# yangdongchao/RSTnet

Measured on NVIDIA H100. Metric: codec_frames_per_s, higher is better.
Workload: dtype f32

## Files before the change

### include/rstnet_b200.h

```cpp
#ifndef RSTNET_B200_H
#define RSTNET_B200_H

#include <stdint.h>

#ifdef __cplusplus
extern "C" {
#endif

typedef void* rstnet_stream_t;

enum { RSTNET_ACT_NONE = 0, RSTNET_ACT_ELU = 1, RSTNET_ACT_GELU = 2 };

int rstnet_version(void);
const char* rstnet_last_error(void);
int64_t rstnet_launch_count(void);
uint32_t rstnet_device_error_flags(int clear);

typedef struct {
  const float* A;
  int64_t a_batch_stride, a_row_stride;
  const float* Wt;
  const float* bias;
  const float* scale;
  const float* R;
// ... 7 lines not shown
} rstnet_gemm_rows_args;
int rstnet_gemm_rows_f32(const rstnet_gemm_rows_args* args, rstnet_stream_t stream);

typedef struct rstnet_tc_plan rstnet_tc_plan;
typedef struct {
  const float* A;
  int64_t a_i_stride, a_o_stride;
  int32_t a_c_extent, a_i_extent, a_o_extent;
  int32_t taps, tap_di, tap_do, o_mul;
  const float* W;
  const float* W_lo;
  int32_t N, Kc;
  int32_t I_out, O_out;
  float* C;
  int64_t c_i_stride, c_o_stride, c_split_stride;
  const float* R;
  int64_t r_i_stride, r_o_stride, r_split_stride;
  const float* bias;
  const float* scale;
  int32_t n_split;
  int32_t pre_act, post_act, precision;
  float* C2;
  int32_t act2;
} rstnet_tc_gemm_desc;
int rstnet_tc_gemm_create(const rstnet_tc_gemm_desc* desc, rstnet_tc_plan** out);
int rstnet_tc_gemm_run(const rstnet_tc_plan* plan, rstnet_stream_t stream);
void rstnet_tc_gemm_destroy(rstnet_tc_plan* plan);
int rstnet_tc_gemm_grid(const rstnet_tc_plan* plan, int32_t* grid_x, int32_t* grid_y, int32_t* tile_n);
typedef struct rstnet_tc_resblock_plan rstnet_tc_resblock_plan;
typedef struct {
  const float* Y;
  int64_t y_i_stride, y_o_stride;
  int32_t channels;
  int32_t I_out, O_out, y_rows;
  const float* W1;
  const float* W1_lo;
  const float* b1;
  const float* W2;
  const float* W2_lo;
  const float* b2;
  float* out;
  int64_t out_i_stride, out_o_stride;
} rstnet_tc_resblock_desc;
int rstnet_tc_resblock_create(const rstnet_tc_resblock_desc* desc, rstnet_tc_resblock_plan** out);
int rstnet_tc_resblock_run(const rstnet_tc_resblock_plan* plan, rstnet_stream_t stream);
void rstnet_tc_resblock_destroy(rstnet_tc_resblock_plan* plan);

int rstnet_tf32_split_f32(const float* x, float* hi, float* lo, int64_t n, rstnet_stream_t stream);

int rstnet_conv1d_cin1_f32(const float* x, int64_t x_batch_stride, int64_t x_time_stride, const float* w, const float* bias,
                           float* out, float* out2 , int64_t out_batch_stride,
// ... 131 lines not shown
```

### rstnet_b200/_lib.py

```python
from __future__ import annotations

import ctypes as C
import os

_HERE = os.path.dirname(os.path.abspath(__file__))
LIB_PATH = os.path.join(_HERE, "lib", "librstnet_b200.so")

ACT_NONE, ACT_ELU, ACT_GELU = 0, 1, 2

SYMBOLS = [
    "rstnet_version", "rstnet_last_error", "rstnet_launch_count", "rstnet_device_error_flags",
    "rstnet_gemm_rows_f32", "rstnet_tc_gemm_create", "rstnet_tc_gemm_run", "rstnet_tc_gemm_destroy", "rstnet_tc_gemm_grid",
    "rstnet_tc_resblock_create", "rstnet_tc_resblock_run", "rstnet_tc_resblock_destroy", "rstnet_tf32_split_f32", "rstnet_conv1d_cin1_f32", "rstnet_conv1d_cout1_f32",
    "rstnet_convtr1d_depthwise_f32", "rstnet_rows_fill_f32", "rstnet_rows_copy_table_f32",
    "rstnet_counter_add", "rstnet_layer_norm_f32", "rstnet_rope_kv_append_f32",
    "rstnet_ring_attention_f32", "rstnet_rope_ring_attention_f32", "rstnet_rvq_encode_workspace", "rstnet_rvq_encode_f32",
    "rstnet_rvq_decode_gather_f32",
    "rstnet_skinny_gemm_workspace", "rstnet_skinny_gemm_create", "rstnet_skinny_gemm_create_fused", "rstnet_skinny_gemm_run", "rstnet_skinny_gemm_destroy",
    "rstnet_lm_embed_sum_bf16", "rstnet_lm_embed_rows_bf16", "rstnet_lm_rms_norm_bf16", "rstnet_lm_rope_kv_append_bf16",
    "rstnet_lm_rope_pair_kv_append_bf16",
    "rstnet_lm_ring_decode_attention_bf16", "rstnet_lm_silu_mul_bf16", "rstnet_lm_depth_attention_bf16",
    "rstnet_resample_f32", "rstnet_lm_delay_cache_in", "rstnet_lm_delay_cache_out", "rstnet_counter_add_rows",
    "rstnet_lm_cross_entropy_bf16", "rstnet_rows_fill_tail_f32", "rstnet_lm_sample_params_bf16",
    "rstnet_lm_rope_kv_append_paged_bf16", "rstnet_lm_paged_decode_attention_bf16",
]

KV_LOG2_PAGE_MIN, KV_LOG2_PAGE_MAX = 4, 12

RESAMPLE_MAX_TABLE_BYTES = 48 * 1024


class GemmRowsArgs(C.Structure):
    _fields_ = [
        ("A", C.c_void_p), ("a_batch_stride", C.c_int64), ("a_row_stride", C.c_int64),
        ("Wt", C.c_void_p), ("bias", C.c_void_p), ("scale", C.c_void_p),
        ("R", C.c_void_p), ("r_batch_stride", C.c_int64), ("r_row_stride", C.c_int64),
        ("C", C.c_void_p), ("c_batch_stride", C.c_int64), ("c_row_stride", C.c_int64),
        ("batch", C.c_int32), ("rows", C.c_int32), ("N", C.c_int32), ("K", C.c_int32),
        ("pre_act", C.c_int32), ("post_act", C.c_int32), ("taps", C.c_int32), ("tap_stride", C.c_int64),
    ]


class TcGemmDesc(C.Structure):
    _fields_ = [
        ("A", C.c_void_p), ("a_i_stride", C.c_int64), ("a_o_stride", C.c_int64),
        ("a_c_extent", C.c_int32), ("a_i_extent", C.c_int32), ("a_o_extent", C.c_int32),
        ("taps", C.c_int32), ("tap_di", C.c_int32), ("tap_do", C.c_int32), ("o_mul", C.c_int32),
        ("W", C.c_void_p), ("W_lo", C.c_void_p), ("N", C.c_int32), ("Kc", C.c_int32), ("I_out", C.c_int32), ("O_out", C.c_int32),
        ("C", C.c_void_p), ("c_i_stride", C.c_int64), ("c_o_stride", C.c_int64), ("c_split_stride", C.c_int64),
        ("R", C.c_void_p), ("r_i_stride", C.c_int64), ("r_o_stride", C.c_int64), ("r_split_stride", C.c_int64),
        ("bias", C.c_void_p), ("scale", C.c_void_p),
        ("n_split", C.c_int32), ("pre_act", C.c_int32), ("post_act", C.c_int32), ("precision", C.c_int32),
        ("C2", C.c_void_p), ("act2", C.c_int32),
    ]


class TcResblockDesc(C.Structure):
    _fields_ = [
        ("Y", C.c_void_p), ("y_i_stride", C.c_int64), ("y_o_stride", C.c_int64),
        ("channels", C.c_int32), ("I_out", C.c_int32), ("O_out", C.c_int32), ("y_rows", C.c_int32),
        ("W1", C.c_void_p), ("W1_lo", C.c_void_p), ("b1", C.c_void_p),
        ("W2", C.c_void_p), ("W2_lo", C.c_void_p), ("b2", C.c_void_p),
        ("out", C.c_void_p), ("out_i_stride", C.c_int64), ("out_o_stride", C.c_int64),
    ]


class RowCopy(C.Structure):
    _fields_ = [("buf", C.c_void_p), ("batch_stride", C.c_int64), ("C", C.c_int32), ("src_row", C.c_int32),
                ("dst_row", C.c_int32), ("nrows", C.c_int32), ("cps", C.c_int32), ("reserved", C.c_int32)]


class RstnetError(RuntimeError):
    pass


_lib = None
# ... 4 lines not shown
    if _lib is not None:
        return _lib
    if not os.path.exists(LIB_PATH):
        raise RstnetError(
            f"{LIB_PATH} not found: the CUDA extension is not built. Run `python -m rstnet_b200.build` "
            "(there is no CPU fallback).")
    from . import build as _build
    stamp = os.path.join(os.path.dirname(LIB_PATH), "build.sha256")
    if os.path.isdir(_build.CSRC) and (not os.path.exists(stamp) or open(stamp).read().strip() != _build._digest()):
        raise RstnetError(
            f"{LIB_PATH} is stale (built from different sources than rstnet_b200/csrc + include/). "
            "Run `python -m rstnet_b200.build`.")
    L = C.CDLL(LIB_PATH)
    vp, i32, i64, f32 = C.c_void_p, C.c_int32, C.c_int64, C.c_float
    L.rstnet_version.restype = C.c_int
    L.rstnet_last_error.restype = C.c_char_p
    L.rstnet_launch_count.restype = i64
    L.rstnet_gemm_rows_f32.argtypes = [C.POINTER(GemmRowsArgs), vp]
    L.rstnet_tc_gemm_create.argtypes = [C.POINTER(TcGemmDesc), C.POINTER(C.c_void_p)]
    L.rstnet_tc_gemm_run.argtypes = [vp, vp]
    L.rstnet_tc_gemm_destroy.argtypes = [vp]
    L.rstnet_tc_gemm_destroy.restype = None
    L.rstnet_tc_gemm_grid.argtypes = [vp, C.POINTER(i32), C.POINTER(i32), C.POINTER(i32)]
    L.rstnet_tc_resblock_create.argtypes = [C.POINTER(TcResblockDesc), C.POINTER(C.c_void_p)]
    L.rstnet_tc_resblock_run.argtypes = [vp, vp]
    L.rstnet_tc_resblock_destroy.argtypes = [vp]
    L.rstnet_tc_resblock_destroy.restype = None
    L.rstnet_tf32_split_f32.argtypes = [vp, vp, vp, i64, vp]
    L.rstnet_conv1d_cin1_f32.argtypes = [vp, i64, i64, vp, vp, vp, vp, i64, i64, i32, i32, i32, i32, i32, i32, vp]
    L.rstnet_conv1d_cout1_f32.argtypes = [vp, i64, i64, vp, vp, vp, i64, i32, i32, i32, i32, vp]
    L.rstnet_convtr1d_depthwise_f32.argtypes = [vp, i64, i64, vp, vp, i64, i64, i32, i32, i32, i32, vp]
    L.rstnet_rows_fill_f32.argtypes = [vp, i64, i32, i32, i32, i32, i32, i32, vp, i32, i32, vp]
    L.rstnet_rows_fill_tail_f32.argtypes = [vp, i64, i32, i32, i32, i32, i32, vp, i64, i32, vp]
    L.rstnet_rows_copy_table_f32.argtypes = [vp, i32, i32, vp, vp]
    L.rstnet_counter_add.argtypes = [vp, i64, i32, vp, vp]
    L.rstnet_layer_norm_f32.argtypes = [vp, i64, vp, vp, vp, i32, i32, i32, f32, vp]
    L.rstnet_rope_kv_append_f32.argtypes = [vp, i64, i64, vp, vp, i32, vp, i32, i32, i32, i32, i32, vp]
    L.rstnet_ring_attention_f32.argtypes = [vp, i64, i64, vp, vp, i32, vp, i64, i64, i32, i32, i32, i32, i32, i32, i32, vp]
    L.rstnet_rope_ring_attention_f32.argtypes = [vp, i64, i64, vp, vp, i32, vp, vp, i64, i64, i32, i32, i32, i32, i32, i32, vp]
    L.rstnet_rvq_encode_workspace.argtypes = [i64, i32, i32, i32]
    L.rstnet_rvq_encode_workspace.restype = i64
    L.rstnet_rvq_encode_f32.argtypes = [vp, i64, vp, vp, vp, vp, vp, i64, i32, i32, i32, i32, i32, i32, vp]
    L.rstnet_rvq_decode_gather_f32.argtypes = [vp, vp, vp, i64, i32, i32, i32, i32, i32, i32, vp]
    L.rstnet_skinny_gemm_workspace.argtypes = [i32, i32, i32]
    L.rstnet_skinny_gemm_workspace.restype = i64
    L.rstnet_skinny_gemm_create.argtypes = [vp, vp, vp, vp, vp, i32, i32, i32, i32, C.POINTER(C.c_void_p)]
# ... 42 lines not shown
```

### rstnet_b200/csrc/gemm_tc.cu

```cuda
#include <cstdlib>

#include "common.cuh"
#include "tc_common.cuh"
#include "../../include/rstnet_b200.h"

namespace rstnet {
extern void count_launch();
using namespace tc;

constexpr int TC_BM = 128;
constexpr int TC_BKE = 32;
constexpr int TC_A_BYTES = TC_BM * 128;
constexpr int TC_CONSUMER_WARPS = 8;
constexpr int TC_THREADS = 32 * TC_CONSUMER_WARPS + 32;
constexpr int TC_CHUNK_STAGES = 4;

struct TcParams {
  float* C;
  float* C2;
  int act2;
  long long c_i_stride, c_o_stride, c_split_stride;
  const float* R;
  long long r_i_stride, r_o_stride, r_split_stride;
  const float* bias;
  const float* scale;
  int n_split;
  int I_out, O_out, N, Kc;
  int taps, tap_di, tap_do, o_mul, kchunks;
  int pre_act, post_act, i_tiles;
  int m_tiles, n_tiles;
};

template <int BN, int PREC>
struct TcCfg {
  static constexpr bool SPLIT = PREC == 0;
  static constexpr int B_BYTES = BN * 128;
  static constexpr int STAGE_BYTES = TC_A_BYTES + B_BYTES * (SPLIT ? 2 : 1);
  static constexpr int STAGES = (200 * 1024 / STAGE_BYTES) > 8 ? 8 : (200 * 1024 / STAGE_BYTES);
  static constexpr int SMEM_BYTES = STAGES * STAGE_BYTES + 1024  + 256 ;
};

__device__ __forceinline__ float tf32_rna(float x) {
  const uint32_t u = __float_as_uint(x);
  return __uint_as_float((x != x ? u | 0x00400000u : u + 0x1000u) & 0xFFFFE000u);
}
__device__ __forceinline__ float tf32_rna_lo(float x, float hi) {
  const float d = x - hi;
  return d != d ? 0.f : __uint_as_float((__float_as_uint(d) + 0x1000u) & 0xFFFFE000u);
}

__device__ __forceinline__ float act_tc(float x, int act) {
  if (act == ACT_ELU) return elu_fast(x);
  if (act == ACT_GELU) return gelu_f(x);
  return x;
}

template <bool SPLIT, bool PRE_ELU>
__device__ __forceinline__ void tc_build_a(uint32_t st, uint32_t a_row, uint32_t a_sw, uint32_t (&ah)[4][4], uint32_t (&al)[4][4]) {
#pragma unroll
  for (int k = 0; k < 4; ++k) {
#pragma unroll
    for (int e = 0; e < 4; ++e) {
// ... 134 lines not shown
          if (p.scale) {
            const float2 ss = *reinterpret_cast<const float2*>(p.scale + n);
            v.x *= ss.x; v.y *= ss.y;
          }
          long long coff = n, roff = n;
          if (p.n_split > 0) {
            const int j = n / p.n_split, co = n % p.n_split;
            coff = (long long)j * p.c_split_stride + co;
            roff = (long long)j * p.r_split_stride + co;
          }
          if (rrow) {
            const float2 rr = *reinterpret_cast<const float2*>(rrow + roff);
            v.x += rr.x; v.y += rr.y;
          }
          if (crow2)
            *reinterpret_cast<float2*>(crow2 + coff) = make_float2(act_tc(v.x, p.act2), act_tc(v.y, p.act2));
          *reinterpret_cast<float2*>(crow + coff) = make_float2(act_tc(v.x, p.post_act), act_tc(v.y, p.post_act));
        }
      }
    }
  }
}

constexpr int RB_B_BYTES = 64 * 128;
constexpr int RB_STAGE_BYTES = TC_A_BYTES + 2 * RB_B_BYTES;
constexpr int RB_STAGES = 6;

struct RbParams {
  float* out;
  long long o_i_stride, o_o_stride;
  const float* b1;
  const float* b2;
  int I_out, i_tiles, m_tiles;
};

template <int C>
struct RbCfg {
  static constexpr int N1 = C / 2;
  static constexpr int KCH = C / 32;
  static constexpr int P1 = 3 * KCH;
  static constexpr int NS = C / 64;
  static constexpr int K2 = N1 / 32;
  static constexpr int H_BYTES = K2 * TC_A_BYTES;
  static constexpr int SMEM_BYTES = RB_STAGES * RB_STAGE_BYTES + H_BYTES + 1024  + 256 ;
  static constexpr bool ring_ok() {
    for (int j = 0; j < NS; ++j)
// ... 178 lines not shown
                                  CUtensorMapL2promotion, CUtensorMapFloatOOBfill);

static EncodeTiledFn get_encode_fn() {
  static EncodeTiledFn fn = nullptr;
  if (!fn) {
    void* p = nullptr;
    cudaDriverEntryPointQueryResult q;
    if (cudaGetDriverEntryPoint("cuTensorMapEncodeTiled", &p, cudaEnableDefault, &q) == cudaSuccess && p) fn = (EncodeTiledFn)p;
  }
  return fn;
}

}
using namespace rstnet;

struct rstnet_tc_plan {
  CUtensorMap tmA, tmW, tmWlo;
  TcParams p;
  dim3 grid;
  int bn, prec;
};

template <int BN, int PREC, bool PRE_ELU>
static int tc_launch(const rstnet_tc_plan* pl, cudaStream_t st) {
  using Cfg = TcCfg<BN, PREC>;
  static unsigned long long attr = 0;
  smem_optin(gemm_tc_kernel<BN, PREC, PRE_ELU>, Cfg::SMEM_BYTES, attr);
  gemm_tc_kernel<BN, PREC, PRE_ELU><<<pl->grid, TC_THREADS, Cfg::SMEM_BYTES, st>>>(pl->tmA, pl->tmW, pl->tmWlo, pl->p);
  count_launch();
  return check_launch("gemm_tc");
}

extern "C" int rstnet_tc_gemm_create(const rstnet_tc_gemm_desc* d, rstnet_tc_plan** out) {
  RSTNET_REQUIRE(d && out, "tc_gemm_create: null argument");
  RSTNET_REQUIRE(d->A && d->W && d->C, "tc_gemm_create: null tensor pointer");
  RSTNET_REQUIRE(d->precision != 0 || d->W_lo, "tc_gemm_create: precision 0 (3xTF32) needs W_lo");
  RSTNET_REQUIRE(d->Kc > 0 && d->Kc % TC_BKE == 0, "tc_gemm_create: Kc (%d) must be a multiple of %d", d->Kc, TC_BKE);
  RSTNET_REQUIRE(d->N > 0 && d->N % 4 == 0, "tc_gemm_create: N (%d) must be a multiple of 4", d->N);
  RSTNET_REQUIRE(d->taps >= 1 && d->I_out > 0 && d->O_out > 0, "tc_gemm_create: bad shape");
  RSTNET_REQUIRE(d->precision == 0 || d->precision == 1, "tc_gemm_create: precision must be 0 (3xTF32) or 1 (TF32)");
  RSTNET_REQUIRE(d->pre_act == ACT_NONE || d->pre_act == ACT_ELU, "tc_gemm_create: pre_act must be NONE or ELU (got %d)", d->pre_act);
  RSTNET_REQUIRE((uintptr_t)d->A % 16 == 0 && (uintptr_t)d->W % 16 == 0 && (uintptr_t)d->C % 16 == 0 &&
                     d->a_i_stride % 4 == 0 && d->a_o_stride % 4 == 0 && d->c_i_stride % 4 == 0 && d->c_o_stride % 4 == 0 &&
                     d->c_split_stride % 4 == 0 && d->n_split % 4 == 0,
                 "tc_gemm_create: 16-byte alignment required");
  EncodeTiledFn enc = get_encode_fn();
  RSTNET_REQUIRE(enc != nullptr, "tc_gemm_create: cuTensorMapEncodeTiled unavailable (no CUDA driver?)");
  rstnet_tc_plan* pl = new rstnet_tc_plan();
  const int N = d->N;
  const int sms = sm_count();
  pl->bn = N >= 64 ? 64 : 32;
  const int i_tiles = ceil_div(d->I_out, TC_BM);
  {
    const long long mt = (long long)i_tiles * d->O_out;
    const long long t64 = mt * ceil_div(N, 64), t32 = mt * ceil_div(N, 32);
    if (pl->bn == 64 && ((t32 + sms - 1) / sms) * 2 <= ((t64 + sms - 1) / sms) * 3) pl->bn = 32;
  }
  pl->prec = d->precision;
  {
    cuuint64_t gdim[3] = {(cuuint64_t)d->a_c_extent, (cuuint64_t)d->a_i_extent, (cuuint64_t)d->a_o_extent};
    cuuint64_t gstr[2] = {(cuuint64_t)d->a_i_stride * 4, (cuuint64_t)d->a_o_stride * 4};
    cuuint32_t box[3] = {TC_BKE, TC_BM, 1};
    cuuint32_t estr[3] = {1, 1, 1};
    CUresult r = enc(&pl->tmA, CU_TENSOR_MAP_DATA_TYPE_FLOAT32, 3, (void*)d->A, gdim, gstr, box, estr, CU_TENSOR_MAP_INTERLEAVE_NONE,
                     CU_TENSOR_MAP_SWIZZLE_128B, CU_TENSOR_MAP_L2_PROMOTION_L2_128B, CU_TENSOR_MAP_FLOAT_OOB_FILL_NONE);
    if (r != CUDA_SUCCESS) {
      delete pl;
      set_error("tc_gemm_create: cuTensorMapEncodeTiled(A) failed with %d", (int)r);
      return 3;
    }
  }
  {
    cuuint64_t gdim[2] = {(cuuint64_t)d->taps * d->Kc, (cuuint64_t)N};
    cuuint64_t gstr[1] = {(cuuint64_t)d->taps * d->Kc * 4};
    cuuint32_t box[2] = {TC_BKE, (cuuint32_t)pl->bn};
    cuuint32_t estr[2] = {1, 1};
    CUresult r = enc(&pl->tmW, CU_TENSOR_MAP_DATA_TYPE_FLOAT32, 2, (void*)d->W, gdim, gstr, box, estr, CU_TENSOR_MAP_INTERLEAVE_NONE,
                     CU_TENSOR_MAP_SWIZZLE_128B, CU_TENSOR_MAP_L2_PROMOTION_L2_256B, CU_TENSOR_MAP_FLOAT_OOB_FILL_NONE);
    if (r == CUDA_SUCCESS && d->W_lo)
      r = enc(&pl->tmWlo, CU_TENSOR_MAP_DATA_TYPE_FLOAT32, 2, (void*)d->W_lo, gdim, gstr, box, estr, CU_TENSOR_MAP_INTERLEAVE_NONE,
              CU_TENSOR_MAP_SWIZZLE_128B, CU_TENSOR_MAP_L2_PROMOTION_L2_256B, CU_TENSOR_MAP_FLOAT_OOB_FILL_NONE);
    else
      pl->tmWlo = pl->tmW;
    if (r != CUDA_SUCCESS) {
      delete pl;
      set_error("tc_gemm_create: cuTensorMapEncodeTiled(W) failed with %d", (int)r);
      return 3;
    }
  }
  TcParams& p = pl->p;
  p.C2 = d->C2; p.act2 = d->act2;
  p.C = d->C; p.c_i_stride = d->c_i_stride; p.c_o_stride = d->c_o_stride; p.c_split_stride = d->c_split_stride;
  p.R = d->R; p.r_i_stride = d->r_i_stride; p.r_o_stride = d->r_o_stride; p.r_split_stride = d->r_split_stride;
  p.bias = d->bias; p.scale = d->scale; p.n_split = d->n_split;
  p.I_out = d->I_out; p.O_out = d->O_out; p.N = N; p.Kc = d->Kc;
  p.taps = d->taps; p.tap_di = d->tap_di; p.tap_do = d->tap_do; p.o_mul = d->o_mul; p.kchunks = d->Kc / TC_BKE;
  p.pre_act = d->pre_act; p.post_act = d->post_act; p.i_tiles = i_tiles;
  p.m_tiles = i_tiles * d->O_out;
  p.n_tiles = ceil_div(N, pl->bn);
  const long long tiles = (long long)p.m_tiles * p.n_tiles;
  pl->grid = dim3((unsigned)(tiles < sms ? tiles : sms));
  *out = pl;
  return 0;
}

extern "C" int rstnet_tc_gemm_run(const rstnet_tc_plan* pl, rstnet_stream_t stream) {
  RSTNET_REQUIRE(pl != nullptr, "tc_gemm_run: null plan");
  cudaStream_t st = (cudaStream_t)stream;
  const bool elu = pl->p.pre_act == ACT_ELU;
  if (pl->prec == 0) {
    if (pl->bn == 64) return elu ? tc_launch<64, 0, true>(pl, st) : tc_launch<64, 0, false>(pl, st);
    return elu ? tc_launch<32, 0, true>(pl, st) : tc_launch<32, 0, false>(pl, st);
  }
  if (pl->bn == 64) return elu ? tc_launch<64, 1, true>(pl, st) : tc_launch<64, 1, false>(pl, st);
  return elu ? tc_launch<32, 1, true>(pl, st) : tc_launch<32, 1, false>(pl, st);
}

extern "C" void rstnet_tc_gemm_destroy(rstnet_tc_plan* pl) { delete pl; }

struct rstnet_tc_resblock_plan {
  CUtensorMap tmY, tmW1, tmW1lo, tmW2, tmW2lo;
  RbParams p;
  dim3 grid;
  int channels;
// ... 54 lines not shown

template <int Cc>
static int rb_launch(const rstnet_tc_resblock_plan* pl, cudaStream_t st) {
  constexpr int smem = RbCfg<Cc>::SMEM_BYTES;
  static unsigned long long attr = 0;
  smem_optin(resblock_tc_kernel<Cc>, smem, attr);
  resblock_tc_kernel<Cc><<<pl->grid, TC_THREADS, smem, st>>>(pl->tmY, pl->tmW1, pl->tmW1lo, pl->tmW2, pl->tmW2lo, pl->p);
  count_launch();
  return check_launch("tc_resblock");
}

extern "C" int rstnet_tc_resblock_run(const rstnet_tc_resblock_plan* pl, rstnet_stream_t stream) {
  RSTNET_REQUIRE(pl != nullptr, "tc_resblock_run: null plan");
  cudaStream_t st = (cudaStream_t)stream;
  return pl->channels == 64 ? rb_launch<64>(pl, st) : rb_launch<128>(pl, st);
}

extern "C" void rstnet_tc_resblock_destroy(rstnet_tc_resblock_plan* pl) { delete pl; }
extern "C" int rstnet_tc_gemm_grid(const rstnet_tc_plan* pl, int32_t* gx, int32_t* gy, int32_t* bn) {
  if (!pl) return 1;
  *gx = pl->p.m_tiles; *gy = pl->p.n_tiles; *bn = pl->bn;
  return 0;
}

namespace rstnet {
__global__ void tf32_split_kernel(const float* __restrict__ x, float* __restrict__ hi, float* __restrict__ lo, long long n) {
  for (long long i = (long long)blockIdx.x * blockDim.x + threadIdx.x; i < n; i += (long long)gridDim.x * blockDim.x) {
    const float v = x[i], h = tf32_rna(v);
    hi[i] = h;
    lo[i] = tf32_rna_lo(v, h);
  }
}
}

extern "C" int rstnet_tf32_split_f32(const float* x, float* hi, float* lo, int64_t n, rstnet_stream_t stream) {
  RSTNET_REQUIRE(x && hi && lo, "tf32_split: null pointer");
  if (n <= 0) return 0;
  int g = ceil_div(n, 256);
  if (g > sm_count() * 8) g = sm_count() * 8;
  rstnet::tf32_split_kernel<<<g, 256, 0, (cudaStream_t)stream>>>(x, hi, lo, n);
  count_launch();
  return check_launch("tf32_split");
}
```

### rstnet_b200/csrc/tc_common.cuh

```cuda
#pragma once
#include <cuda.h>
#include <cuda_runtime.h>
#include <cstdint>

namespace rstnet {
namespace tc {

__device__ __forceinline__ uint32_t smem_u32(const void* p) { return static_cast<uint32_t>(__cvta_generic_to_shared(p)); }

__device__ __forceinline__ bool elect_one() {
  uint32_t pred = 0;
  asm volatile(
      "{\n\t.reg .b32 rx;\n\t.reg .pred px;\n\t"
      "elect.sync rx|px, 0xFFFFFFFF;\n\t"
      "selp.u32 %0, 1, 0, px;\n\t}"
      : "=r"(pred));
  return pred != 0;
}

__device__ __forceinline__ void mbar_init(uint64_t* bar, uint32_t count) {
  asm volatile("mbarrier.init.shared::cta.b64 [%0], %1;" ::"r"(smem_u32(bar)), "r"(count));
}
__device__ __forceinline__ void fence_barrier_init() { asm volatile("fence.mbarrier_init.release.cluster;" ::: "memory"); }
__device__ __forceinline__ void mbar_arrive(uint64_t* bar) {
  asm volatile("{\n\t.reg .b64 st;\n\tmbarrier.arrive.shared::cta.b64 st, [%0];\n\t}" ::"r"(smem_u32(bar)) : "memory");
}
__device__ __forceinline__ void mbar_arrive_expect_tx(uint64_t* bar, uint32_t bytes) {
  asm volatile("{\n\t.reg .b64 st;\n\tmbarrier.arrive.expect_tx.shared::cta.b64 st, [%0], %1;\n\t}" ::"r"(smem_u32(bar)), "r"(bytes)
               : "memory");
}
__device__ __forceinline__ bool mbar_try_wait(uint64_t* bar, uint32_t parity) {
  uint32_t ok;
  asm volatile(
      "{\n\t.reg .pred p;\n\t"
      "mbarrier.try_wait.parity.shared::cta.b64 p, [%1], %2;\n\t"
      "selp.u32 %0, 1, 0, p;\n\t}"
      : "=r"(ok)
      : "r"(smem_u32(bar)), "r"(parity)
      : "memory");
  return ok != 0;
}
__device__ __forceinline__ void mbar_wait(uint64_t* bar, uint32_t parity) {
  while (!mbar_try_wait(bar, parity)) {
  }
}

__device__ __forceinline__ void tma_prefetch_desc(const CUtensorMap* m) {
  asm volatile("prefetch.tensormap [%0];" ::"l"(reinterpret_cast<uint64_t>(m)) : "memory");
}
__device__ __forceinline__ void tma_load_2d(void* dst, const CUtensorMap* m, uint64_t* bar, int c0, int c1) {
  asm volatile("cp.async.bulk.tensor.2d.shared::cta.global.mbarrier::complete_tx::bytes [%0], [%1, {%3, %4}], [%2];" ::"r"(
                   smem_u32(dst)),
               "l"(reinterpret_cast<uint64_t>(m)), "r"(smem_u32(bar)), "r"(c0), "r"(c1)
               : "memory");
}
__device__ __forceinline__ void tma_load_3d(void* dst, const CUtensorMap* m, uint64_t* bar, int c0, int c1, int c2) {
  asm volatile("cp.async.bulk.tensor.3d.shared::cta.global.mbarrier::complete_tx::bytes [%0], [%1, {%3, %4, %5}], [%2];" ::"r"(
                   smem_u32(dst)),
               "l"(reinterpret_cast<uint64_t>(m)), "r"(smem_u32(bar)), "r"(c0), "r"(c1), "r"(c2)
               : "memory");
}
__device__ __forceinline__ void named_bar_sync(int id, int nthreads) { asm volatile("bar.sync %0, %1;" ::"r"(id), "r"(nthreads) : "memory"); }

__device__ __forceinline__ uint64_t gmma_desc_sw128(uint32_t saddr) {
  uint64_t d = 0;
  d |= (uint64_t)((saddr & 0x3FFFF) >> 4);
  d |= (uint64_t)1 << 16;
// ... 101 lines not shown
```

### rstnet_b200/ops.py

```python
from __future__ import annotations

import ctypes as C
from typing import Optional

import torch

from . import _lib
from ._lib import ACT_ELU, ACT_GELU, ACT_NONE, GemmRowsArgs, RowCopy, TcGemmDesc


def _stream() -> int:
    return torch.cuda.current_stream().cuda_stream


def _p(t: Optional[torch.Tensor]) -> Optional[int]:
    return None if t is None else t.data_ptr()


def _cuda(*ts):
    for t in ts:
        if t is not None and not t.is_cuda:
            raise _lib.RstnetError("rstnet_b200 ops need CUDA tensors (there is no CPU path)")


# ... 12 lines not shown
    a.r_batch_stride, a.r_row_stride = r_bs, r_rs
    a.C = C_.data_ptr() + 4 * c_off
    a.c_batch_stride, a.c_row_stride = c_bs, c_rs
    a.batch, a.rows, a.N, a.K = batch, rows, N, K
    a.pre_act, a.post_act = pre_act, post_act
    a.taps, a.tap_stride = taps, tap_stride
    _lib.check(_lib.lib().rstnet_gemm_rows_f32(C.byref(a), _stream()), "gemm_rows_f32")


def tf32_split(w: torch.Tensor):
    _cuda(w)
    w = w.contiguous()
    both = torch.empty((2,) + tuple(w.shape), dtype=w.dtype, device=w.device)
    hi, lo = both[0], both[1]
    _lib.check(_lib.lib().rstnet_tf32_split_f32(w.data_ptr(), hi.data_ptr(), lo.data_ptr(), w.numel(), _stream()), "tf32_split")
    return hi, lo


class TcGemm:

    def __init__(self, A, a_off, a_i_stride, a_o_stride, a_c_extent, a_i_extent, a_o_extent, W, Kc, C_, c_off, c_i_stride,
                 c_o_stride, I_out, O_out, *, taps=1, tap_di=0, tap_do=0, o_mul=1, bias=None, scale=None, R=None, r_off=0,
                 r_i_stride=0, r_o_stride=0, n_split=0, c_split_stride=0, r_split_stride=0, pre_act=ACT_NONE,
                 post_act=ACT_NONE, precision=0, W_lo=None, C2=None, c2_off=0, act2=ACT_NONE):
        _cuda(A, W, C_, bias, scale, R, W_lo)
        N, Ktot = W.shape
        if precision == 0 and W_lo is None:
            W, W_lo = tf32_split(W)
        assert Ktot == taps * Kc, (Ktot, taps, Kc)
        d = TcGemmDesc()
        d.A = A.data_ptr() + 4 * a_off
        d.a_i_stride, d.a_o_stride = a_i_stride, a_o_stride
        d.a_c_extent, d.a_i_extent, d.a_o_extent = a_c_extent, a_i_extent, a_o_extent
        d.taps, d.tap_di, d.tap_do, d.o_mul = taps, tap_di, tap_do, o_mul
        d.W, d.W_lo, d.N, d.Kc, d.I_out, d.O_out = W.data_ptr(), _p(W_lo), N, Kc, I_out, O_out
        d.C = C_.data_ptr() + 4 * c_off
        d.c_i_stride, d.c_o_stride, d.c_split_stride = c_i_stride, c_o_stride, c_split_stride
        d.R = None if R is None else R.data_ptr() + 4 * r_off
        d.r_i_stride, d.r_o_stride, d.r_split_stride = r_i_stride, r_o_stride, r_split_stride
        d.bias, d.scale = _p(bias), _p(scale)
        d.n_split, d.pre_act, d.post_act, d.precision = n_split, pre_act, post_act, precision
        d.C2 = None if C2 is None else C2.data_ptr() + 4 * c2_off
        d.act2 = act2
        self._keep = (A, W, W_lo, C_, bias, scale, R, C2)
        self.flops = 2.0 * I_out * O_out * N * Ktot
        in_rows = min(a_o_extent, O_out * o_mul + (taps - 1) * max(tap_do, 0))
        n_out = I_out * O_out * N
        self.bytes = 4.0 * (a_c_extent * a_i_extent * in_rows + (2 if W_lo is not None else 1) * N * Ktot
                            + n_out * (2 if C2 is not None else 1) + (n_out if R is not None else 0))
        self._h = C.c_void_p()
        _lib.check(_lib.lib().rstnet_tc_gemm_create(C.byref(d), C.byref(self._h)), "tc_gemm_create")

    def run(self):
        _lib.check(_lib.lib().rstnet_tc_gemm_run(self._h, _stream()), "tc_gemm_run")

    def __del__(self):
        h = getattr(self, "_h", None)
        if h:
            try:
                _lib.lib().rstnet_tc_gemm_destroy(h)
            except Exception:
                pass
            self._h = None


class TcResblock:

    def __init__(self, Y, y_off, y_i_stride, y_o_stride, y_rows, I_out, O_out, W1, W1_lo, b1, W2, W2_lo, b2, out, out_off,
                 out_i_stride, out_o_stride):
        _cuda(Y, W1, W1_lo, b1, W2, W2_lo, b2, out)
        Cc = W2.shape[0]
        assert tuple(W1.shape) == (Cc // 2, 3 * Cc) and tuple(W2.shape) == (Cc, Cc // 2), (W1.shape, W2.shape)
        d = _lib.TcResblockDesc()
        d.Y = Y.data_ptr() + 4 * y_off
        d.y_i_stride, d.y_o_stride = y_i_stride, y_o_stride
        d.channels, d.I_out, d.O_out, d.y_rows = Cc, I_out, O_out, y_rows
        d.W1, d.W1_lo, d.b1 = W1.data_ptr(), W1_lo.data_ptr(), b1.data_ptr()
# ... 124 lines not shown
```

Measured before the change: 42970.

## Add cluster-based split-K tensor-core GEMM with DSMEM partial-sum handoff

Adds a split-K variant of the TF32 tensor-core GEMM that launches thread-block clusters, where each CTA in a cluster handles interleaved K blocks and passes partial accumulators to the next rank through distributed shared memory with st.async and cluster mbarriers. The plan picks the split factor automatically from a cost model when there are too few output tiles to fill the SMs. The aim is better SM utilisation for small-M/N, large-K codec GEMMs. It costs extra shared memory, serialised handoffs between ranks, and cluster launch overhead.

```diff
diff --git a/include/rstnet_b200.h b/include/rstnet_b200.h
--- a/include/rstnet_b200.h
+++ b/include/rstnet_b200.h
@@ -53,11 +53,13 @@
   int32_t pre_act, post_act, precision;
   float* C2;
   int32_t act2;
+  int32_t k_split;
 } rstnet_tc_gemm_desc;
 int rstnet_tc_gemm_create(const rstnet_tc_gemm_desc* desc, rstnet_tc_plan** out);
 int rstnet_tc_gemm_run(const rstnet_tc_plan* plan, rstnet_stream_t stream);
 void rstnet_tc_gemm_destroy(rstnet_tc_plan* plan);
 int rstnet_tc_gemm_grid(const rstnet_tc_plan* plan, int32_t* grid_x, int32_t* grid_y, int32_t* tile_n);
+int rstnet_tc_gemm_split(const rstnet_tc_plan* plan, int32_t* k_split, int32_t* clusters);
 typedef struct rstnet_tc_resblock_plan rstnet_tc_resblock_plan;
 typedef struct {
   const float* Y;
diff --git a/rstnet_b200/_lib.py b/rstnet_b200/_lib.py
--- a/rstnet_b200/_lib.py
+++ b/rstnet_b200/_lib.py
@@ -11,6 +11,7 @@
 SYMBOLS = [
     "rstnet_version", "rstnet_last_error", "rstnet_launch_count", "rstnet_device_error_flags",
     "rstnet_gemm_rows_f32", "rstnet_tc_gemm_create", "rstnet_tc_gemm_run", "rstnet_tc_gemm_destroy", "rstnet_tc_gemm_grid",
+    "rstnet_tc_gemm_split",
     "rstnet_tc_resblock_create", "rstnet_tc_resblock_run", "rstnet_tc_resblock_destroy", "rstnet_tf32_split_f32", "rstnet_conv1d_cin1_f32", "rstnet_conv1d_cout1_f32",
     "rstnet_convtr1d_depthwise_f32", "rstnet_rows_fill_f32", "rstnet_rows_copy_table_f32",
     "rstnet_counter_add", "rstnet_layer_norm_f32", "rstnet_rope_kv_append_f32",
@@ -51,7 +52,7 @@
         ("R", C.c_void_p), ("r_i_stride", C.c_int64), ("r_o_stride", C.c_int64), ("r_split_stride", C.c_int64),
         ("bias", C.c_void_p), ("scale", C.c_void_p),
         ("n_split", C.c_int32), ("pre_act", C.c_int32), ("post_act", C.c_int32), ("precision", C.c_int32),
-        ("C2", C.c_void_p), ("act2", C.c_int32),
+        ("C2", C.c_void_p), ("act2", C.c_int32), ("k_split", C.c_int32),
     ]
 
 
@@ -102,6 +103,7 @@
     L.rstnet_tc_gemm_destroy.argtypes = [vp]
     L.rstnet_tc_gemm_destroy.restype = None
     L.rstnet_tc_gemm_grid.argtypes = [vp, C.POINTER(i32), C.POINTER(i32), C.POINTER(i32)]
+    L.rstnet_tc_gemm_split.argtypes = [vp, C.POINTER(i32), C.POINTER(i32)]
     L.rstnet_tc_resblock_create.argtypes = [C.POINTER(TcResblockDesc), C.POINTER(C.c_void_p)]
     L.rstnet_tc_resblock_run.argtypes = [vp, vp]
     L.rstnet_tc_resblock_destroy.argtypes = [vp]
diff --git a/rstnet_b200/csrc/gemm_tc.cu b/rstnet_b200/csrc/gemm_tc.cu
--- a/rstnet_b200/csrc/gemm_tc.cu
+++ b/rstnet_b200/csrc/gemm_tc.cu
@@ -14,6 +14,7 @@
 constexpr int TC_CONSUMER_WARPS = 8;
 constexpr int TC_THREADS = 32 * TC_CONSUMER_WARPS + 32;
 constexpr int TC_CHUNK_STAGES = 4;
+constexpr int tc_split_block(int bn) { return bn == 64 ? 1 : 2; }
 
 struct TcParams {
   float* C;
@@ -29,6 +30,7 @@
   int taps, tap_di, tap_do, o_mul, kchunks;
   int pre_act, post_act, i_tiles;
   int m_tiles, n_tiles;
+  int ksplit;
 };
 
 template <int BN, int PREC>
@@ -38,6 +40,10 @@
   static constexpr int STAGE_BYTES = TC_A_BYTES + B_BYTES * (SPLIT ? 2 : 1);
   static constexpr int STAGES = (200 * 1024 / STAGE_BYTES) > 8 ? 8 : (200 * 1024 / STAGE_BYTES);
   static constexpr int SMEM_BYTES = STAGES * STAGE_BYTES + 1024  + 256 ;
+  static constexpr int XBUF_BYTES = 32 * TC_CONSUMER_WARPS * (BN / 2) * 4;
+  static constexpr int SMEM_SPLIT_BYTES = SMEM_BYTES + XBUF_BYTES;
+  static_assert((2 * STAGES + 2 * TC_CONSUMER_WARPS) * 8 <= 256, "barriers overflow their 256 bytes");
+  static_assert(SMEM_SPLIT_BYTES <= 227 * 1024, "split form exceeds the shared memory of an SM");
 };
 
 __device__ __forceinline__ float tf32_rna(float x) {
@@ -218,6 +224,193 @@
   }
 }
 
+static_assert(tc_split_block(32) <= 2 && tc_split_block(64) <= 2, "the split kernel keeps at most one chunk value aside");
+template <int BN, int PREC, bool PRE_ELU>
+__global__ void __launch_bounds__(TC_THREADS, 1)
+gemm_tc_split_kernel(const __grid_constant__ CUtensorMap tmA, const __grid_constant__ CUtensorMap tmW,
+               const __grid_constant__ CUtensorMap tmWlo, const TcParams p) {
+  using Cfg = TcCfg<BN, PREC>;
+  constexpr int S = Cfg::STAGES;
+  constexpr int CH = TC_CHUNK_STAGES;
+  constexpr int NR = BN / 2;
+  extern __shared__ uint8_t smem_raw[];
+  uint8_t* smem = smem_raw + ((1024u - (smem_u32(smem_raw) & 1023u)) & 1023u);
+  uint64_t* full = reinterpret_cast<uint64_t*>(smem + S * Cfg::STAGE_BYTES);
+  uint64_t* empty = full + S;
+  uint64_t* xfull = empty + S;
+  uint64_t* xfree = xfull + TC_CONSUMER_WARPS;
+  uint8_t* xbuf = smem + S * Cfg::STAGE_BYTES + 256;
+  const int warp = threadIdx.x / 32, lane = threadIdx.x % 32;
+  const int total_k = p.taps * p.kchunks;
+  const int total_tiles = p.m_tiles * p.n_tiles;
+  constexpr int BLK = tc_split_block(BN) * TC_CHUNK_STAGES;
+  const int ks = p.ksplit, rank = blockIdx.x % ks;
+  const int tile0 = blockIdx.x / ks, tile_step = gridDim.x / ks;
+
+  if (threadIdx.x == 0) {
+    for (int s = 0; s < S; ++s) {
+      mbar_init(&full[s], 1);
+      mbar_init(&empty[s], TC_CONSUMER_WARPS);
+    }
+    if (ks > 1)
+      for (int w = 0; w < TC_CONSUMER_WARPS; ++w) {
+        mbar_init(&xfull[w], 1);
+        mbar_init(&xfree[w], 1);
+        mbar_arrive_expect_tx(&xfull[w], Cfg::XBUF_BYTES / TC_CONSUMER_WARPS);
+      }
+    fence_barrier_init();
+  }
+  __syncthreads();
+  if (ks > 1) cluster_sync();
+
+  if (warp == TC_CONSUMER_WARPS) {
+    if (elect_one()) {
+      tma_prefetch_desc(&tmA);
+      tma_prefetch_desc(&tmW);
+      if (Cfg::SPLIT) tma_prefetch_desc(&tmWlo);
+      int g = 0;
+      for (int t = tile0; t < total_tiles; t += tile_step) {
+        const int nt = t % p.n_tiles, mt = t / p.n_tiles;
+        const int i0 = (mt % p.i_tiles) * TC_BM, ot = mt / p.i_tiles, n0 = nt * BN;
+        for (int k0 = rank * BLK; k0 < total_k; k0 += ks * BLK) {
+          const int kend = total_k - k0 < BLK ? total_k : k0 + BLK;
+          for (int kit = k0; kit < kend; ++kit, ++g) {
+            const int s = g % S;
+            mbar_wait(&empty[s], ((g / S) & 1) ^ 1);
+            const int tap = kit / p.kchunks, kc = kit % p.kchunks;
+            uint8_t* st = smem + s * Cfg::STAGE_BYTES;
+            mbar_arrive_expect_tx(&full[s], Cfg::STAGE_BYTES);
+            tma_load_3d(st, &tmA, &full[s], kc * TC_BKE, i0 + tap * p.tap_di, ot * p.o_mul + tap * p.tap_do);
+            tma_load_2d(st + TC_A_BYTES, &tmW, &full[s], kit * TC_BKE, n0);
+            if (Cfg::SPLIT) tma_load_2d(st + TC_A_BYTES + Cfg::B_BYTES, &tmWlo, &full[s], kit * TC_BKE, n0);
+          }
+        }
+      }
+    }
+    return;
+  }
+
+  const int wg = warp / 4, wq = warp % 4, gq = lane / 4, tq = lane % 4;
+  const int r0 = wg * 64 + wq * 16 + gq;
+  const uint32_t a_row = (uint32_t)r0 * 128u + (uint32_t)tq * 4u, a_sw = (uint32_t)(r0 & 7);
+  const uint32_t smem0 = smem_u32(smem);
+  float acc[NR], d0[NR], d1[NR];
+#pragma unroll
+  for (int j = 0; j < NR; ++j) d0[j] = d1[j] = 0.f;
+  const uint32_t x_off = (uint32_t)(warp * (NR / 4) * 32 + lane) * 16u;
+  const uint32_t xbuf_in = smem_u32(xbuf) + x_off;
+  const uint32_t xbuf_next = ks > 1 ? cluster_map(xbuf, (rank + 1) % ks) + x_off : 0u;
+  const uint32_t xfull_next = ks > 1 ? cluster_map(&xfull[warp], (rank + 1) % ks) : 0u;
+  const uint32_t xfree_prev = ks > 1 ? cluster_map(&xfree[warp], (rank + ks - 1) % ks) : 0u;
+  const int last_rank = ((total_k - 1) / BLK) % ks;
+  int n_in = 0, n_out = 0;
+  int g = 0;
+  for (int t = tile0; t < total_tiles; t += tile_step) {
+    const int nt = t % p.n_tiles, mt = t / p.n_tiles;
+    const int i0 = (mt % p.i_tiles) * TC_BM, ot = mt / p.i_tiles, n0 = nt * BN;
+#pragma unroll
+    for (int j = 0; j < NR; ++j) acc[j] = 0.f;
+    for (int b0 = rank * BLK; b0 < total_k; b0 += ks * BLK) {
+      const int kend = total_k - b0 < BLK ? total_k : b0 + BLK;
+      float pend[NR];
+      for (int k0 = b0; k0 < kend; k0 += CH) {
+        const int nst = kend - k0 < CH ? kend - k0 : CH;
+        for (int u = 0; u < nst; ++u, ++g) {
+          const int s = g % S;
+          mbar_wait(&full[s], (g / S) & 1);
+          const uint32_t st = smem0 + (uint32_t)(s * Cfg::STAGE_BYTES);
+          uint32_t ah[4][4], al[4][4];
+          tc_build_a<Cfg::SPLIT, PRE_ELU>(st, a_row, a_sw, ah, al);
+          const uint64_t db = gmma_desc_sw128(st + TC_A_BYTES);
+          const uint64_t dbl = gmma_desc_sw128(st + TC_A_BYTES + Cfg::B_BYTES);
+          wgmma_fence();
+          tc_mma_stage<BN, Cfg::SPLIT>(d0, d1, ah, al, db, dbl, u == 0);
+          wgmma_commit();
+          wgmma_wait<0>();
+          __syncwarp();
+          if (lane == 0) mbar_arrive(&empty[s]);
+        }
+        fence_acc(d0);
+        if (Cfg::SPLIT) fence_acc(d1);
+        if (tc_split_block(BN) == 2 && k0 + CH < kend) {
+#pragma unroll
+          for (int j = 0; j < NR; ++j) pend[j] = Cfg::SPLIT ? d0[j] + d1[j] : d0[j];
+        }
+      }
+      const bool recv = b0 > 0;
+      if (recv) {
+        mbar_wait_cluster(&xfull[warp], n_in & 1);
+        ++n_in;
+#pragma unroll
+        for (int j = 0; j < NR; j += 4) {
+          float4 v;
+          asm volatile("ld.shared.v4.f32 {%0, %1, %2, %3}, [%4];" : "=f"(v.x), "=f"(v.y), "=f"(v.z), "=f"(v.w)
+                       : "r"(xbuf_in + (uint32_t)(j / 4) * 512u) : "memory");
+          acc[j] = v.x; acc[j + 1] = v.y; acc[j + 2] = v.z; acc[j + 3] = v.w;
+        }
+      }
+      if (tc_split_block(BN) == 2 && kend - b0 > CH) {
+#pragma unroll
+        for (int j = 0; j < NR; ++j) acc[j] += pend[j];
+      }
+#pragma unroll
+      for (int j = 0; j < NR; ++j) acc[j] += Cfg::SPLIT ? d0[j] + d1[j] : d0[j];
+      if (recv) {
+        __syncwarp();
+        if (lane == 0) {
+          mbar_arrive_expect_tx(&xfull[warp], Cfg::XBUF_BYTES / TC_CONSUMER_WARPS);
+          mbar_arrive_cluster(xfree_prev);
+        }
+      }
+      if (kend < total_k) {
+        mbar_wait_cluster(&xfree[warp], (n_out & 1) ^ 1);
+        ++n_out;
+#pragma unroll
+        for (int j = 0; j < NR; j += 4)
+          st_async_v4(xbuf_next + (uint32_t)(j / 4) * 512u, acc[j], acc[j + 1], acc[j + 2], acc[j + 3], xfull_next);
+      }
+    }
+    if (rank != last_rank) continue;
+#pragma unroll
+    for (int h = 0; h < 2; ++h) {
+      const int i = i0 + r0 + 8 * h;
+      if (i >= p.I_out) continue;
+      float* crow = p.C + (long long)ot * p.c_o_stride + (long long)i * p.c_i_stride;
+      float* crow2 = p.C2 ? p.C2 + (long long)ot * p.c_o_stride + (long long)i * p.c_i_stride : nullptr;
+      const float* rrow = p.R ? p.R + (long long)ot * p.r_o_stride + (long long)i * p.r_i_stride : nullptr;
+#pragma unroll
+      for (int b = 0; b < BN / 8; ++b) {
+        const int n = n0 + 8 * b + 2 * tq;
+        if (n < p.N) {
+          float2 v = make_float2(acc[4 * b + 2 * h], acc[4 * b + 2 * h + 1]);
+          if (p.bias) {
+            const float2 bb = *reinterpret_cast<const float2*>(p.bias + n);
+            v.x += bb.x; v.y += bb.y;
+          }
+          if (p.scale) {
+            const float2 ss = *reinterpret_cast<const float2*>(p.scale + n);
+            v.x *= ss.x; v.y *= ss.y;
+          }
+          long long coff = n, roff = n;
+          if (p.n_split > 0) {
+            const int j = n / p.n_split, co = n % p.n_split;
+            coff = (long long)j * p.c_split_stride + co;
+            roff = (long long)j * p.r_split_stride + co;
+          }
+          if (rrow) {
+            const float2 rr = *reinterpret_cast<const float2*>(rrow + roff);
+            v.x += rr.x; v.y += rr.y;
+          }
+          if (crow2)
+            *reinterpret_cast<float2*>(crow2 + coff) = make_float2(act_tc(v.x, p.act2), act_tc(v.y, p.act2));
+          *reinterpret_cast<float2*>(crow + coff) = make_float2(act_tc(v.x, p.post_act), act_tc(v.y, p.post_act));
+        }
+      }
+    }
+  }
+  if (ks > 1) cluster_sync();
+}
+
 constexpr int RB_B_BYTES = 64 * 128;
 constexpr int RB_STAGE_BYTES = TC_A_BYTES + 2 * RB_B_BYTES;
 constexpr int RB_STAGES = 6;
@@ -442,13 +635,81 @@
 };
 
 template <int BN, int PREC, bool PRE_ELU>
+static void tc_split_optin() {
+  static unsigned long long attr = 0;
+  smem_optin(gemm_tc_split_kernel<BN, PREC, PRE_ELU>, TcCfg<BN, PREC>::SMEM_SPLIT_BYTES, attr);
+}
+
+static cudaLaunchConfig_t tc_cluster_config(dim3 grid, int ksplit, int smem, cudaStream_t st, cudaLaunchAttribute* attr) {
+  cudaLaunchConfig_t cfg = {};
+  cfg.gridDim = grid;
+  cfg.blockDim = dim3(TC_THREADS);
+  cfg.dynamicSmemBytes = (size_t)smem;
+  cfg.stream = st;
+  attr->id = cudaLaunchAttributeClusterDimension;
+  attr->val.clusterDim.x = (unsigned)ksplit;
+  attr->val.clusterDim.y = 1;
+  attr->val.clusterDim.z = 1;
+  cfg.attrs = attr;
+  cfg.numAttrs = 1;
+  return cfg;
+}
+
+template <int BN, int PREC, bool PRE_ELU>
+static int tc_active_clusters(int ksplit) {
+  using Cfg = TcCfg<BN, PREC>;
+  tc_split_optin<BN, PREC, PRE_ELU>();
+  cudaLaunchAttribute attr;
+  const cudaLaunchConfig_t cfg = tc_cluster_config(dim3((unsigned)(ksplit * sm_count())), ksplit, Cfg::SMEM_SPLIT_BYTES, 0, &attr);
+  int n = 0;
+  if (cudaOccupancyMaxActiveClusters(&n, gemm_tc_split_kernel<BN, PREC, PRE_ELU>, &cfg) != cudaSuccess) {
+    cudaGetLastError();
+    return 0;
+  }
+  return n;
+}
+
+static int tc_active_clusters(int bn, int prec, bool elu, int ksplit) {
+  if (prec == 0) {
+    if (bn == 64) return elu ? tc_active_clusters<64, 0, true>(ksplit) : tc_active_clusters<64, 0, false>(ksplit);
+    return elu ? tc_active_clusters<32, 0, true>(ksplit) : tc_active_clusters<32, 0, false>(ksplit);
+  }
+  if (bn == 64) return elu ? tc_active_clusters<64, 1, true>(ksplit) : tc_active_clusters<64, 1, false>(ksplit);
+  return elu ? tc_active_clusters<32, 1, true>(ksplit) : tc_active_clusters<32, 1, false>(ksplit);
+}
+
+template <int BN, int PREC, bool PRE_ELU>
 static int tc_launch(const rstnet_tc_plan* pl, cudaStream_t st) {
   using Cfg = TcCfg<BN, PREC>;
-  static unsigned long long attr = 0;
-  smem_optin(gemm_tc_kernel<BN, PREC, PRE_ELU>, Cfg::SMEM_BYTES, attr);
-  gemm_tc_kernel<BN, PREC, PRE_ELU><<<pl->grid, TC_THREADS, Cfg::SMEM_BYTES, st>>>(pl->tmA, pl->tmW, pl->tmWlo, pl->p);
+  if (pl->p.ksplit == 1) {
+    static unsigned long long attr = 0;
+    smem_optin(gemm_tc_kernel<BN, PREC, PRE_ELU>, Cfg::SMEM_BYTES, attr);
+    gemm_tc_kernel<BN, PREC, PRE_ELU><<<pl->grid, TC_THREADS, Cfg::SMEM_BYTES, st>>>(pl->tmA, pl->tmW, pl->tmWlo, pl->p);
+  } else {
+    tc_split_optin<BN, PREC, PRE_ELU>();
+    cudaLaunchAttribute attr;
+    const cudaLaunchConfig_t cfg = tc_cluster_config(pl->grid, pl->p.ksplit, Cfg::SMEM_SPLIT_BYTES, st, &attr);
+    cudaLaunchKernelEx(&cfg, gemm_tc_split_kernel<BN, PREC, PRE_ELU>, pl->tmA, pl->tmW, pl->tmWlo, pl->p);
+  }
   count_launch();
   return check_launch("gemm_tc");
+}
+
+constexpr int TC_MAX_SPLIT = 4;
+constexpr int TC_HANDOFF_COST = 6;
+constexpr int TC_SPLIT_LAUNCH_COST = 10;
+
+static long long tc_split_cost(int bn, int ksplit, long long rounds, int total_k) {
+  if (ksplit == 1) return rounds * 2LL * total_k;
+  const int BLK = tc_split_block(bn) * TC_CHUNK_STAGES;
+  int worst = 0, worst_blocks = 0;
+  for (int r = 0; r < ksplit; ++r) {
+    int st = 0, n = 0;
+    for (int b0 = r * BLK; b0 < total_k; b0 += ksplit * BLK, ++n) st += total_k - b0 < BLK ? total_k - b0 : BLK;
+    worst = st > worst ? st : worst;
+    worst_blocks = n > worst_blocks ? n : worst_blocks;
+  }
+  return rounds * (2LL * worst + TC_HANDOFF_COST * worst_blocks + TC_SPLIT_LAUNCH_COST);
 }
 
 extern "C" int rstnet_tc_gemm_create(const rstnet_tc_gemm_desc* d, rstnet_tc_plan** out) {
@@ -460,6 +721,11 @@
   RSTNET_REQUIRE(d->taps >= 1 && d->I_out > 0 && d->O_out > 0, "tc_gemm_create: bad shape");
   RSTNET_REQUIRE(d->precision == 0 || d->precision == 1, "tc_gemm_create: precision must be 0 (3xTF32) or 1 (TF32)");
   RSTNET_REQUIRE(d->pre_act == ACT_NONE || d->pre_act == ACT_ELU, "tc_gemm_create: pre_act must be NONE or ELU (got %d)", d->pre_act);
+  RSTNET_REQUIRE(d->k_split >= 0 && d->k_split <= TC_MAX_SPLIT,
+                 "tc_gemm_create: k_split (%d) must be 0 (automatic), 1 (never) or 2 .. %d", d->k_split, TC_MAX_SPLIT);
+  RSTNET_REQUIRE(d->k_split <= ceil_div(d->taps * (d->Kc / TC_BKE), TC_CHUNK_STAGES),
+                 "tc_gemm_create: k_split (%d) exceeds the %d K chunks of %d stages", d->k_split,
+                 ceil_div(d->taps * (d->Kc / TC_BKE), TC_CHUNK_STAGES), TC_CHUNK_STAGES);
   RSTNET_REQUIRE((uintptr_t)d->A % 16 == 0 && (uintptr_t)d->W % 16 == 0 && (uintptr_t)d->C % 16 == 0 &&
                      d->a_i_stride % 4 == 0 && d->a_o_stride % 4 == 0 && d->c_i_stride % 4 == 0 && d->c_o_stride % 4 == 0 &&
                      d->c_split_stride % 4 == 0 && d->n_split % 4 == 0,
@@ -477,6 +743,28 @@
     if (pl->bn == 64 && ((t32 + sms - 1) / sms) * 2 <= ((t64 + sms - 1) / sms) * 3) pl->bn = 32;
   }
   pl->prec = d->precision;
+  const bool elu = d->pre_act == ACT_ELU;
+  int ksplit = 1, active = 0;
+  if (d->k_split > 1) {
+    ksplit = d->k_split;
+    active = tc_active_clusters(pl->bn, pl->prec, elu, ksplit);
+    if (active <= 0) {
+      delete pl;
+      set_error("tc_gemm_create: no cluster of %d CTAs fits on the device", ksplit);
+      return 1;
+    }
+  } else if (d->k_split == 0) {
+    const int total_k = d->taps * (d->Kc / TC_BKE), nck = ceil_div(total_k, TC_CHUNK_STAGES);
+    const long long tiles = (long long)i_tiles * d->O_out * ceil_div(N, pl->bn);
+    long long best = tc_split_cost(pl->bn, 1, (tiles + sms - 1) / sms, total_k);
+    for (int c = 2; c <= TC_MAX_SPLIT && c <= nck; ++c) {
+      const long long cost = tc_split_cost(pl->bn, c, 1, total_k);
+      if (cost >= best) continue;
+      const int act = tc_active_clusters(pl->bn, pl->prec, elu, c);
+      if (tiles > act) continue;
+      best = cost, ksplit = c, active = act;
+    }
+  }
   {
     cuuint64_t gdim[3] = {(cuuint64_t)d->a_c_extent, (cuuint64_t)d->a_i_extent, (cuuint64_t)d->a_o_extent};
     cuuint64_t gstr[2] = {(cuuint64_t)d->a_i_stride * 4, (cuuint64_t)d->a_o_stride * 4};
@@ -518,8 +806,10 @@
   p.pre_act = d->pre_act; p.post_act = d->post_act; p.i_tiles = i_tiles;
   p.m_tiles = i_tiles * d->O_out;
   p.n_tiles = ceil_div(N, pl->bn);
+  p.ksplit = ksplit;
   const long long tiles = (long long)p.m_tiles * p.n_tiles;
-  pl->grid = dim3((unsigned)(tiles < sms ? tiles : sms));
+  if (ksplit == 1) pl->grid = dim3((unsigned)(tiles < sms ? tiles : sms));
+  else pl->grid = dim3((unsigned)(ksplit * (tiles < active ? tiles : active)));
   *out = pl;
   return 0;
 }
@@ -620,6 +910,12 @@
   *gx = pl->p.m_tiles; *gy = pl->p.n_tiles; *bn = pl->bn;
   return 0;
 }
+extern "C" int rstnet_tc_gemm_split(const rstnet_tc_plan* pl, int32_t* k_split, int32_t* clusters) {
+  RSTNET_REQUIRE(pl && k_split && clusters, "tc_gemm_split: null argument");
+  *k_split = pl->p.ksplit;
+  *clusters = (int32_t)pl->grid.x / pl->p.ksplit;
+  return 0;
+}
 
 namespace rstnet {
 __global__ void tf32_split_kernel(const float* __restrict__ x, float* __restrict__ hi, float* __restrict__ lo, long long n) {
diff --git a/rstnet_b200/csrc/tc_common.cuh b/rstnet_b200/csrc/tc_common.cuh
--- a/rstnet_b200/csrc/tc_common.cuh
+++ b/rstnet_b200/csrc/tc_common.cuh
@@ -43,6 +43,35 @@
 __device__ __forceinline__ void mbar_wait(uint64_t* bar, uint32_t parity) {
   while (!mbar_try_wait(bar, parity)) {
   }
+}
+
+__device__ __forceinline__ uint32_t cluster_map(const void* p, uint32_t rank) {
+  uint32_t r;
+  asm volatile("mapa.shared::cluster.u32 %0, %1, %2;" : "=r"(r) : "r"(smem_u32(p)), "r"(rank));
+  return r;
+}
+__device__ __forceinline__ void st_async_v4(uint32_t addr, float a, float b, float c, float d, uint32_t remote_bar) {
+  asm volatile("st.async.shared::cluster.mbarrier::complete_tx::bytes.v4.f32 [%0], {%1, %2, %3, %4}, [%5];" ::"r"(addr), "f"(a),
+               "f"(b), "f"(c), "f"(d), "r"(remote_bar)
+               : "memory");
+}
+__device__ __forceinline__ void mbar_arrive_cluster(uint32_t remote_bar) {
+  asm volatile("mbarrier.arrive.release.cluster.shared::cluster.b64 _, [%0];" ::"r"(remote_bar) : "memory");
+}
+__device__ __forceinline__ void mbar_wait_cluster(uint64_t* bar, uint32_t parity) {
+  uint32_t ok = 0;
+  while (!ok) {
+    asm volatile(
+        "{\n\t.reg .pred p;\n\t"
+        "mbarrier.try_wait.parity.acquire.cluster.shared::cta.b64 p, [%1], %2;\n\t"
+        "selp.u32 %0, 1, 0, p;\n\t}"
+        : "=r"(ok)
+        : "r"(smem_u32(bar)), "r"(parity)
+        : "memory");
+  }
+}
+__device__ __forceinline__ void cluster_sync() {
+  asm volatile("barrier.cluster.arrive.release;\n\tbarrier.cluster.wait.acquire;" ::: "memory");
 }
 
 __device__ __forceinline__ void tma_prefetch_desc(const CUtensorMap* m) {
diff --git a/rstnet_b200/ops.py b/rstnet_b200/ops.py
--- a/rstnet_b200/ops.py
+++ b/rstnet_b200/ops.py
@@ -58,7 +58,7 @@
     def __init__(self, A, a_off, a_i_stride, a_o_stride, a_c_extent, a_i_extent, a_o_extent, W, Kc, C_, c_off, c_i_stride,
                  c_o_stride, I_out, O_out, *, taps=1, tap_di=0, tap_do=0, o_mul=1, bias=None, scale=None, R=None, r_off=0,
                  r_i_stride=0, r_o_stride=0, n_split=0, c_split_stride=0, r_split_stride=0, pre_act=ACT_NONE,
-                 post_act=ACT_NONE, precision=0, W_lo=None, C2=None, c2_off=0, act2=ACT_NONE):
+                 post_act=ACT_NONE, precision=0, W_lo=None, C2=None, c2_off=0, act2=ACT_NONE, k_split=0):
         _cuda(A, W, C_, bias, scale, R, W_lo)
         N, Ktot = W.shape
         if precision == 0 and W_lo is None:
@@ -78,6 +78,7 @@
         d.n_split, d.pre_act, d.post_act, d.precision = n_split, pre_act, post_act, precision
         d.C2 = None if C2 is None else C2.data_ptr() + 4 * c2_off
         d.act2 = act2
+        d.k_split = k_split
         self._keep = (A, W, W_lo, C_, bias, scale, R, C2)
         self.flops = 2.0 * I_out * O_out * N * Ktot
         in_rows = min(a_o_extent, O_out * o_mul + (taps - 1) * max(tap_do, 0))
@@ -89,6 +90,11 @@
 
     def run(self):
         _lib.check(_lib.lib().rstnet_tc_gemm_run(self._h, _stream()), "tc_gemm_run")
+
+    def split(self):
+        ks, cl = C.c_int32(), C.c_int32()
+        _lib.check(_lib.lib().rstnet_tc_gemm_split(self._h, C.byref(ks), C.byref(cl)), "tc_gemm_split")
+        return ks.value, cl.value
 
     def __del__(self):
         h = getattr(self, "_h", None)
```

After: 43950, median of 6. 2.3% higher.
